# Koellewe/nano-dpow

Hardware: AMD Instinct MI355X
Metric: Gnonce/s blake2b-64 per GPU & 8-GPU node; p50 time-to-work at fffffff8 (higher is better)
Workload: dtype u64

## Files before the change

include/nanopow.h:

```cpp
#ifndef NANOPOW_H
#define NANOPOW_H

#include <stdint.h>

#ifdef __cplusplus
extern "C" {
#endif

#define NPOW_OK 0
#define NPOW_CANCELLED 1
#define NPOW_EXHAUSTED 2
#define NPOW_PENDING 3
#define NPOW_TOO_LATE 4
#define NPOW_ERR_NOT_INITIALISED (-1)
#define NPOW_ERR_NO_DEVICE (-2)
#define NPOW_ERR_BAD_ARGUMENT (-3)
#define NPOW_ERR_HIP (-4)
#define NPOW_ERR_INVALID_WORK (-5)
#define NPOW_ERR_CAPACITY (-6)
#define NPOW_ERR_INTERNAL (-7)

#define NPOW_ABI_VERSION 7

#define NPOW_RESERVE_MIN 0xfffff00000000000ull
// ... 195 lines not shown
  uint64_t launches;
  uint64_t launches_cut;
  uint64_t held_us;
  uint64_t moves;
} npow_range_share_info;

int npow_ticket_share(uint64_t ticket, npow_range_share_info* out);

int npow_values(int device, const uint8_t root[32], uint64_t start, uint64_t count, uint64_t* values_out);

int npow_values_path(int device, const uint8_t root[32], uint64_t start, uint64_t count, int path,
                     uint64_t* values_out);

int npow_values_pairs(int device, const uint8_t* roots, const uint64_t* nonces, uint32_t n,
                      uint64_t* values_out);

int npow_set_tuning(uint32_t iters_per_launch, uint32_t poll_interval, uint32_t blocks_per_cu);

int npow_set_pool_tuning(uint32_t budget_us, uint32_t blocks_per_cu);

int npow_device_stats_get(int device, npow_device_stats* out);
int npow_device_stats_get_sized(int device, npow_device_stats* out, uint64_t size);
int npow_device_stats_reset(int device);

const char* npow_version(void);
int npow_abi_version(void);

#ifdef __cplusplus
}
#endif

#endif
```

nano-dpow_amd/csrc/npow_engine.cpp:

```cpp
#include <hip/hip_runtime.h>

#include <pthread.h>
#include <time.h>

#include <algorithm>
#include <cstddef>
#include <exception>
#include <chrono>
#include <cstdio>
#include <cstdlib>
#include <cstring>
#include <deque>
#include <memory>
#include <mutex>
#include <string>
#include <thread>
#include <vector>

#include "npow_host.h"

namespace npow {

namespace {
thread_local std::string t_err;
// ... 495 lines not shown
  out->stale_missing = d.stale_missing;
  out->stale_gpu_delay_us = d.stale_gpu_delay_us;
  out->linger_ms = d.linger_ms;
  out->promotions = d.promotions;
  return NPOW_OK;
}

int npow_device_stats_get(int device, npow_device_stats* out) try {
  if (!out) return fail(NPOW_ERR_BAD_ARGUMENT, "out is required");
  npow_device_stats full;
  if (int rc = stats_fill(device, &full)) return rc;
  memcpy(out, &full, offsetof(npow_device_stats, kills_relayed));
  return NPOW_OK;
} catch (...) { return guard_exception(); }

int npow_device_stats_get_sized(int device, npow_device_stats* out, uint64_t size) try {
  if (!out || size == 0) return fail(NPOW_ERR_BAD_ARGUMENT, "out and size > 0 are required");
  npow_device_stats full;
  if (int rc = stats_fill(device, &full)) return rc;
  memcpy(out, &full, std::min<uint64_t>(size, sizeof(full)));
  return NPOW_OK;
} catch (...) { return guard_exception(); }

int npow_device_stats_reset(int device) try {
  if (int rc = check_init()) return rc;
  if (device < 0 || device >= (int)g_devs.size()) return fail(NPOW_ERR_BAD_ARGUMENT, "bad device");
  Device& d = *g_devs[device];
  settle_stats(d);
  const double cpu = worker_cpu_ms(d);
  std::lock_guard<std::mutex> g(d.stats_mu);
  d.launches = d.nonces = d.invalid = d.early = d.early_mismatch = d.yields = d.dyn = d.kills_relayed = d.late = 0;
  d.promotions = d.idle_gaps = d.watcher_decisions = d.stale_drains = d.linger_relays = d.stale_late = d.stale_missing = 0;
  d.idle_ms = d.linger_ms = d.stale_gpu_delay_us = 0.0;
  d.kernel_ms = 0.0;
  d.clk_ticks = d.clk_ref_ticks = 0.0;
  d.stats_t0 = std::chrono::steady_clock::now();
  d.worker_cpu0_ms = cpu;
  return NPOW_OK;
} catch (...) { return guard_exception(); }

int npow_search(const uint8_t root[32], uint64_t threshold, uint64_t start, uint64_t device_mask,
                uint64_t max_nonces_per_device, const volatile uint32_t* cancel, uint64_t* nonce_out,
                uint64_t* value_out, uint64_t* nonces_done) try {
  if (int rc = check_init()) return rc;
  if (!root || !nonce_out) return fail(NPOW_ERR_BAD_ARGUMENT, "root and nonce_out are required");
  uint64_t ticket = 0;
  if (int rc = pool_submit(root, threshold, start, device_mask, max_nonces_per_device, cancel, &ticket)) return rc;
  return pool_wait(ticket, -1, nonce_out, value_out, nonces_done);
} catch (...) { return guard_exception(); }

int npow_search_batch(const uint8_t* roots, const uint64_t* thresholds, uint32_t n, uint64_t device_mask,
                      uint64_t max_nonces_per_root, const volatile uint32_t* const* cancel, uint64_t* nonces_out,
                      uint64_t* values_out, int32_t* status_out, uint64_t* nonces_done) try {
  if (int rc = check_init()) return rc;
  if (nonces_done) *nonces_done = 0;
  if (n == 0) return NPOW_OK;
// ... 405 lines not shown
```

nano-dpow_amd/csrc/npow_host.h:

```cpp
#pragma once
#include <hip/hip_runtime.h>
#include <pthread.h>

#include <atomic>
#include <condition_variable>
#include <chrono>
#include <memory>
#include <mutex>
#include <string>
#include <thread>
#include <vector>

#include "../../include/nanopow.h"
#include "npow_blake2b.h"
#include "npow_internal.h"

namespace npow {

int fail(int code, const std::string& msg);
const std::string& last_error();

#define HIPTRY(expr)                                                                        \
  do {                                                                                      \
    hipError_t e_ = (expr);                                                                 \
// ... 17 lines not shown
  HostMailbox* mb_dev = nullptr;
  uint64_t* d_out = nullptr;
  hipEvent_t ev_start[kEventRing] = {};
  hipEvent_t ev_stop[kEventRing] = {};
  std::mutex mu;
  std::atomic<int> tasks_waiting{0};
  PoolDevState* pst = nullptr;
  PoolMailbox* pmb = nullptr;
  PoolMailbox* pmb_dev = nullptr;
  PoolTable* d_tab[kEventRing] = {};
  PoolTable* h_tab[kEventRing] = {};
  unsigned long long* h_done = nullptr;
  hipEvent_t ev_done[kMaxSlots] = {};
  hipStream_t hit_stream = nullptr;
  unsigned long long* h_hit_ring = nullptr;
  unsigned long long* h_hit_n = nullptr;
  uint64_t* h_hits = nullptr;
  std::thread worker;
  std::mutex stats_mu;
  uint64_t launches = 0, nonces = 0, invalid = 0;
  uint64_t early = 0, early_mismatch = 0;
  uint64_t yields = 0, dyn = 0;
  uint64_t linger_ends = 0;
  uint64_t promotions = 0;
  std::atomic<int> counted_inflight{0};
  uint64_t kills_relayed = 0;
  uint64_t late = 0;
  uint64_t watcher_decisions = 0;
  uint64_t stale_drains = 0;
  uint64_t stale_late = 0;
  uint64_t stale_missing = 0;
  double stale_gpu_delay_us = 0.0;
  uint64_t linger_relays = 0;
  double linger_ms = 0.0;
  double idle_ms = 0.0;
  uint64_t idle_gaps = 0;
  std::atomic<bool> worker_busy{false};
  std::atomic<int> active_slots{0};
  std::mutex wake_mu;
  std::condition_variable wake_cv;
  uint64_t wake_seq = 0;
  std::atomic<uint64_t> armed_mask{0};
  std::atomic<uint64_t> armed_gen[kMaxSlots] = {};
  std::atomic<const volatile uint32_t*> armed_cancel[kMaxSlots] = {};
  std::atomic<double> armed_spin_until[kMaxSlots] = {};
  std::mutex armed_mu;
// ... 110 lines not shown
```

nano-dpow_amd/csrc/npow_internal.h:

```cpp
#pragma once
#include <stddef.h>
#include <stdint.h>
#include <hip/hip_runtime.h>

#include "npow_blake2b.h"
#include "npow_weights.h"
#include "npow_claims.h"
#include "npow_dense.h"
#include "npow_hash_asm.inc"
#include "npow_hash_asm_lockstep_ld.inc"

namespace npow {

constexpr int kBlock = 256;
constexpr int kLsWaves = 8;
constexpr int kLsBlock = kLsWaves * 64;
static_assert(kDenseWaves == (uint32_t)kLsWaves, "npow_dense.h: one block per wave of a workgroup");
constexpr int kLsGroups = 4;

enum class Mode : int { kSweep = 1, kValues = 2, kValuesSeq = 3 };

struct LaunchArgs {
  uint64_t u[NPOW_ASM_N_UNIFORMS];
  uint64_t threshold;
// ... 181 lines not shown
  PoolReserve reserve[kMaxSlots];
  alignas(64) uint64_t ctl;
  alignas(64) uint64_t kills;
  alignas(64) PoolClk clk[kPoolRing][kClkWaves];
#ifdef NPOW_DIAG_TIMES
  uint64_t diag_join[1024];
#endif
};

struct PoolShape {
  int grid;
  uint32_t units() const { return (uint32_t)grid; }
  uint64_t own(uint32_t e, uint32_t n, uint32_t iters) const {
    return dense_own(units(), n, e, iters);
  }
  uint64_t full(uint32_t iters) const { return dense_full(units(), iters); }
  uint32_t launch_iters(uint32_t iters) const { return iters > 1 ? iters / 2 : 1u; }
};

hipError_t launch_task(Mode mode, int grid, hipStream_t stream, const LaunchArgs& a, DevState* st,
                       HostMailbox* mb, uint64_t* out);
hipError_t launch_pool(hipStream_t stream, int grid, const PoolTable* tab, bool bounded, PoolDevState* st,
                       PoolMailbox* mb);
hipError_t launch_pool_arg(hipStream_t stream, int grid, const PoolTable& host_tab, bool bounded, PoolDevState* st,
                           PoolMailbox* mb);
inline void fill_uniforms(LaunchArgs& a, const RootPrecomp& pre) { npow_asm_uniforms(pre.m, a.u); }

hipError_t launch_pairs(int grid, hipStream_t stream, const uint64_t* roots_words, const uint64_t* nonces,
                        uint32_t n, uint64_t* out);

}
```

nano-dpow_amd/csrc/npow_kernel.hip:

```cpp
#include <hip/hip_runtime.h>
#include <stdint.h>
#include <string.h>

#include "npow_internal.h"

namespace npow {

__device__ __forceinline__ uint64_t pack(uint32_t lo, uint32_t hi) { return ((uint64_t)hi << 32) | lo; }

__device__ __forceinline__ uint64_t rotr32(uint64_t x) {
  return pack((uint32_t)(x >> 32), (uint32_t)x);
}
template <int N>
__device__ __forceinline__ uint64_t rotr_lt32(uint64_t x) {
  const uint32_t lo = (uint32_t)x, hi = (uint32_t)(x >> 32);
  return pack(__builtin_amdgcn_alignbit(hi, lo, N), __builtin_amdgcn_alignbit(lo, hi, N));
}
__device__ __forceinline__ uint64_t rotr63(uint64_t x) {
  const uint32_t lo = (uint32_t)x, hi = (uint32_t)(x >> 32);
  return pack(__builtin_amdgcn_alignbit(lo, hi, 31), __builtin_amdgcn_alignbit(hi, lo, 31));
}

template <int I>
__device__ __forceinline__ uint64_t add_msg(uint64_t a, uint64_t nonce, const uint64_t (&m)[4]) {
// ... 384 lines not shown
                                             uint64_t wn, uint64_t wv) {
  if (__hip_atomic_fetch_max(&st->slot[slot].dead, (unsigned long long)gen, __ATOMIC_RELAXED,
                             __HIP_MEMORY_SCOPE_AGENT) < gen) {
    PoolWin* pw = &mb->win[slot];
    __hip_atomic_store(&pw->nonce, wn, __ATOMIC_RELAXED, __HIP_MEMORY_SCOPE_SYSTEM);
    __hip_atomic_store(&pw->value, wv, __ATOMIC_RELAXED, __HIP_MEMORY_SCOPE_SYSTEM);
    __hip_atomic_store(&pw->t, __builtin_amdgcn_s_memrealtime(), __ATOMIC_RELAXED, __HIP_MEMORY_SCOPE_SYSTEM);
    __hip_atomic_store(&pw->gen, gen, __ATOMIC_RELEASE, __HIP_MEMORY_SCOPE_SYSTEM);
  }
}

__device__ __forceinline__ void ls2_publish_reserve(PoolDevState* st, PoolMailbox* mb, uint32_t slot, uint64_t gen,
                                                    uint64_t rn, uint64_t rv) {
  const unsigned long long key = pool_reserve_key(gen, rv);
  if (__hip_atomic_fetch_max(&st->reserve_best[slot], key, __ATOMIC_RELAXED, __HIP_MEMORY_SCOPE_AGENT) < key) {
    PoolReserve* pr = &mb->reserve[slot];
    __hip_atomic_store(&pr->nonce, rn, __ATOMIC_RELAXED, __HIP_MEMORY_SCOPE_SYSTEM);
    __hip_atomic_store(&pr->gen, gen, __ATOMIC_RELEASE, __HIP_MEMORY_SCOPE_SYSTEM);
  }
}

constexpr uint32_t kNoEntry = 0xffffffffu;
typedef const __attribute__((address_space(4))) PoolEntry ConstEntry;
__device__ __forceinline__ ConstEntry* ls2_entry(const PoolTable* tab, const PoolMailbox* mb, uint32_t e) {
  const PoolEntry* p = e < tab->n ? &tab->e[e] : &mb->dyn[(tab->dyn_base + (e - tab->n)) % kDynRing].e;
  return (ConstEntry*)(uintptr_t)p;
}
struct EntryHdr {
  uint64_t gen;
  uint32_t slot, bounded, wsh, bg;
};
__device__ __forceinline__ EntryHdr ls2_hdr(const PoolTable* tab, PoolMailbox* mb, uint32_t e) {
  if (e < tab->n) {
    ConstEntry* q = (ConstEntry*)(uintptr_t)&tab->e[e];
    return EntryHdr{q->gen, q->slot, q->bounded, q->wsh, q->bg};
  }
  PoolEntry* q = &mb->dyn[(tab->dyn_base + (e - tab->n)) % kDynRing].e;
  const uint32_t w = __hip_atomic_load(&q->wsh, __ATOMIC_RELAXED, __HIP_MEMORY_SCOPE_SYSTEM);
  return EntryHdr{__hip_atomic_load(&q->gen, __ATOMIC_RELAXED, __HIP_MEMORY_SCOPE_SYSTEM),
                  __hip_atomic_load(&q->slot, __ATOMIC_RELAXED, __HIP_MEMORY_SCOPE_SYSTEM),
                  __hip_atomic_load(&q->bounded, __ATOMIC_RELAXED, __HIP_MEMORY_SCOPE_SYSTEM), w,
                  (w & kWshBg) ? 1u : 0u};
}
__device__ __forceinline__ uint64_t ls2_ctl(PoolMailbox* mb) {
  return __hip_atomic_load(&mb->ctl, __ATOMIC_RELAXED, __HIP_MEMORY_SCOPE_SYSTEM);
}
// ... 354 lines not shown
      if (ok) atomicAdd(&ph->moves[q->slot], 1ull);
    }
    if (__builtin_amdgcn_readfirstlane(ok)) return pick;
  }
  return kNoEntry;
}

__device__ __noinline__ uint32_t ls2_claimed_start(const PoolTable* tab, uint32_t g, uint32_t G, uint32_t csum) {
  const uint32_t lane = __builtin_amdgcn_mbcnt_hi(~0u, __builtin_amdgcn_mbcnt_lo(~0u, 0u));
  const uint32_t n = tab->n < (uint32_t)kMaxSlots ? tab->n : (uint32_t)kMaxSlots;
  const uint32_t r = pool_claimed_pos(g, csum, G, pool_claimed_pad_mult(tab->pad));
  ConstEntry* const le = (ConstEntry*)(uintptr_t)&tab->e[lane < n ? lane : 0u];
  uint32_t acc = lane < n ? 8u >> (le->wsh & 3u) : 0u;
#pragma unroll
  for (int m = 1; m < 64; m <<= 1) {
    const uint32_t o = __shfl_up(acc, m);
    if (lane >= (uint32_t)m) acc += o;
  }
  const uint32_t k = (uint32_t)__builtin_popcountll(__ballot(lane < n && acc <= r));
  return k < n ? k : n - 1u;
}

constexpr uint32_t kPollStride = 0x9E3779B9u;

template <bool BOUNDED>
__device__ __forceinline__ void pool_body_ls2(const PoolTable* __restrict__ tab, PoolDevState* __restrict__ st,
                                              PoolMailbox* __restrict__ mb, const uint64_t t_start) {
  __shared__ uint32_t s_stop[3];
  __shared__ uint32_t s_flag[kLsWaves];
  __shared__ uint32_t s_next;
  __shared__ uint32_t s_done[kLsWaves];
  __shared__ uint32_t s_seen;
  const uint32_t lane = threadIdx.x & 63;
  const uint32_t wv = __builtin_amdgcn_readfirstlane(threadIdx.x >> 6);
  const uint32_t g = blockIdx.x, G = gridDim.x;
  const uint32_t w = g * kLsWaves + wv;
  const uint32_t n = tab->n, iters = tab->iters;
  if (threadIdx.x < 3) s_stop[threadIdx.x] = ~0u;
  const bool counted = tab->counted != 0;
  if (wv == 0) {
    if (lane == 0) {
      s_seen = 0;
      s_over = 0;
    }
    uint32_t first;
    if (n == 0) {
      first = kNoEntry;
    } else if (counted) {
      uint32_t e0 = g % n;
      if constexpr (BOUNDED) {
        const uint32_t cs = pool_claimed_pad_sum(tab->pad);
        if (cs) e0 = ls2_claimed_start(tab, g, G, cs);
      }
      first = ls2_pick(tab, st, mb, e0, true, &s_seen);
    } else {
      ConstEntry* pe = ls2_entry(tab, mb, g % n);
      first = load_dead(st, pe->slot) < pe->gen ? g % n : kNoEntry;
    }
    if (lane == 0) s_next = first;
  }
  __syncthreads();

  uint32_t e = __builtin_amdgcn_readfirstlane(__hip_atomic_load(&s_next, __ATOMIC_RELAXED, __HIP_MEMORY_SCOPE_WORKGROUP));
  uint32_t seg = 0, it = 0;
  uint32_t pc = w;
  bool end = false;
  for (;;) {
  for (;;) {
    if (e == kNoEntry) break;
    const PoolEntry* pe = (const PoolEntry*)ls2_entry(tab, mb, e);
    PoolCursor c;
    pool_load_ls(pe, c, g, wv, G, n, e, iters);
#ifdef NPOW_DIAG_TIMES
    if (wv == 0 && lane == 0) {
      const uint64_t tj = __builtin_amdgcn_s_memrealtime();
      __hip_atomic_store(&mb->fin[c.slot].t_join, tj, __ATOMIC_RELAXED, __HIP_MEMORY_SCOPE_SYSTEM);
      __hip_atomic_store(&mb->diag_join[g & 1023], tj, __ATOMIC_RELAXED, __HIP_MEMORY_SCOPE_SYSTEM);
    }
#endif
    pc = w;
    const uint32_t sw = seg % 3;
    const uint32_t poll_mask = tab->poll_mask, budget = tab->budget;
    unsigned long long* const dead_p = &st->slot[c.slot].dead;
    uint32_t b = it * c.K + c.j;
    uint64_t nonce = c.base + ((uint64_t)b << 6) + lane;
    uint64_t step = (uint64_t)c.K << 6;
    uint32_t done = 0;
    __shared__ uint32_t s_it;
    if constexpr (BOUNDED) {
      if ((c.bounded & kEntryClaim) && wv == 0 && lane == 0) s_it = it;
    }
    for (;;) {
    if constexpr (BOUNDED) {
      if (c.bounded & kEntryClaim) {
        __shared__ uint32_t s_claim;
        if (wv == 0 && lane == 0)
          s_claim = ls2_claim(tab, st, mb, pe,
                              __hip_atomic_load(&s_stop[sw], __ATOMIC_RELAXED, __HIP_MEMORY_SCOPE_WORKGROUP), t_start);
        __syncthreads();
        const uint32_t ci = __builtin_amdgcn_readfirstlane(
            __hip_atomic_load(&s_claim, __ATOMIC_RELAXED, __HIP_MEMORY_SCOPE_WORKGROUP));
        __syncthreads();
        if (ci == kNoEntry) break;
        c.K = kLsWaves;
        c.j = wv;
        step = (uint64_t)kLsWaves << 6;
        it = claim_row_first(ci);
        c.it_end = claim_row_end(c.last_b / kLsWaves + 1u, ci);
        b = it * kLsWaves + wv;
        nonce = c.base + ((uint64_t)b << 6) + lane;
      }
    }
    while (it < c.it_end) {
      const uint32_t verdict = __hip_atomic_load(&s_stop[sw], __ATOMIC_RELAXED, __HIP_MEMORY_SCOPE_WORKGROUP);
      const uint64_t dead = __hip_atomic_load(dead_p, __ATOMIC_RELAXED, __HIP_MEMORY_SCOPE_AGENT);
      const uint32_t v = (uint32_t)__builtin_amdgcn_readfirstlane(verdict);
      if (v != ~0u && (v >> 2) <= it) {
        end = (v & 3u) == 0;
        break;
      }
      const uint32_t it0 = it;
      const uint32_t pc0 = pc;
      const uint64_t thr = c.threshold, gen = c.gen;
      const uint64_t value = npow_asm_work_value_lockstep_ld(nonce, c.up);
      ++it;
      pc += kPollStride;
      bool hit = value >= thr;
      if constexpr (BOUNDED) {
        const uint32_t in_lanes = b < c.last_b ? 64u : (b == c.last_b ? c.tail : 0u);
        hit = hit && lane < in_lanes;
        done += in_lanes;
      } else {
        done += 64;
      }
      uint64_t hits = __ballot(hit);
      if constexpr (BOUNDED) {
        if (__builtin_expect(hits != 0, 0) && (c.bounded & kEntryCollect)) {
          c.threshold = ls2_collect(tab, st, c.up, hits, hit, nonce, value, thr, lane);
          hits = 0;
        }
      }
      uint32_t why = 0u;
      if (__builtin_expect(hits != 0, 0)) {
        ConstEntry* ce = (ConstEntry*)(uintptr_t)c.up;
        asm volatile("" : "+s"(ce));
        const uint32_t wslot = ce->slot;
        const uint64_t wgen = ce->gen;
        PoolFloor* const fl = &mb->floor[wslot];
        const uint64_t fgen = __hip_atomic_load(&fl->gen, __ATOMIC_RELAXED, __HIP_MEMORY_SCOPE_SYSTEM);
        ls2_complete();
        const uint64_t ethr = ce->threshold;
        uint64_t cur = ethr;
        if (uni64(fgen) == wgen) {
          const uint64_t fthr = __hip_atomic_load(&fl->threshold, __ATOMIC_RELAXED, __HIP_MEMORY_SCOPE_SYSTEM);
          ls2_complete();
          cur = uni64(fthr);
        }
        const bool armed = ce->reserve != ethr;
        if (cur > thr) {
          if (!armed) c.threshold = cur;
          const uint64_t keep = hits & __ballot(value >= cur);
          const uint64_t stale = hits & ~keep & __ballot(value >= ethr);
          if (stale != 0 && lane == 0)
            atomicAdd(&st->done[wslot][(blockIdx.x % kPoolDoneShards) * 8 + kStaleWord],
                      (unsigned long long)__builtin_popcountll(stale));
          uint64_t cand = hits & ~keep & ~stale;
          hits = keep;
          if (cand != 0) {
            uint64_t bv = 0, bn = 0;
            do {
              const int cl = __builtin_ctzll(cand);
              cand &= cand - 1;
              const uint64_t cv = readlane64(value, cl);
              if (cv >= bv) {
                bv = cv;
                bn = readlane64(nonce, cl);
              }
            } while (cand != 0);
            if (lane == 0) ls2_publish_reserve(st, mb, wslot, wgen, bn, bv);
          }
        }
        if (hits != 0) {
          why = 2u;
          const int wl = __builtin_ctzll(hits);
          const uint64_t wn = readlane64(nonce, wl), wval = readlane64(value, wl);
          if (lane == 0) ls2_publish_win(st, mb, wslot, wgen, wn, wval);
        }
      }
      if (__builtin_expect((pc0 & poll_mask) == 0, 0)) {
        if (lane == 0) s_flag[wv] = ls2_poll(tab, st, mb, e, &s_seen);
        lds_drain();
        const uint32_t p = __builtin_amdgcn_readfirstlane(
            __hip_atomic_load(&s_flag[wv], __ATOMIC_RELAXED, __HIP_MEMORY_SCOPE_WAVEFRONT));
        why = (p & 2u) ? 2u : (why ? why : (p ? 3u : 0u));
      }
      if (__ballot(dead == gen) != 0) why = 1u;
      const bool late = budget && !c.bounded && (it0 & 3u) == 0 &&
                        (uint32_t)__builtin_amdgcn_s_memrealtime() - (uint32_t)t_start >= budget;
      if (__builtin_expect(why != 0 || late, 0)) {
        if (lane == 0)
          __hip_atomic_fetch_min(&s_stop[sw], (it << 2) | (late ? 0u : why), __ATOMIC_RELAXED,
                                 __HIP_MEMORY_SCOPE_WORKGROUP);
        lds_drain();
      }
      nonce += step;
      b += c.K;
      __builtin_amdgcn_s_barrier();
    }
    if constexpr (BOUNDED) {
      if (c.bounded & kEntryClaim) continue;
    }
    break;
    }
    if (lane == 0) s_done[wv] = done;
    __syncthreads();
    if (wv == 0) {
      uint32_t sum = lane < kLsWaves ? s_done[lane] : 0u;
#pragma unroll
      for (int m = kLsWaves / 2; m >= 1; m >>= 1) sum += __shfl_xor(sum, m);
// ... 12 lines not shown
    if (wv == 0) {
      const uint32_t next = ls2_pick(tab, st, mb, e, false, &s_seen);
      if (lane == 0) {
        s_next = next;
        s_stop[(seg + 1) % 3] = ~0u;
      }
    }
    __syncthreads();
    e = __builtin_amdgcn_readfirstlane(__hip_atomic_load(&s_next, __ATOMIC_RELAXED, __HIP_MEMORY_SCOPE_WORKGROUP));
    ++seg;
  }
  if constexpr (BOUNDED) {
    if (e != kNoEntry || !counted) break;
    __syncthreads();
    if (wv == 0) {
      const uint32_t next = ls2_move_claimed(tab, st, mb, (uint32_t)t_start);
      if (lane == 0) s_next = next;
    }
    __syncthreads();
    e = __builtin_amdgcn_readfirstlane(__hip_atomic_load(&s_next, __ATOMIC_RELAXED, __HIP_MEMORY_SCOPE_WORKGROUP));
    if (e == kNoEntry) break;
    continue;
  }
  if (e != kNoEntry || !tab->linger) break;
  __syncthreads();
  if (wv == 0) {
    const uint32_t next = ls2_linger(tab, st, mb, &s_seen, 0);
    if (lane == 0) s_next = next;
  }
  __syncthreads();
  e = __builtin_amdgcn_readfirstlane(__hip_atomic_load(&s_next, __ATOMIC_RELAXED, __HIP_MEMORY_SCOPE_WORKGROUP));
  if (e == kNoEntry) break;
  }
  if (!counted && wv == 0) ls2_exit(tab, st, mb, G, g);
  clk_end_ls2(tab, mb, t_start, wv);
}

template <bool BOUNDED>
__global__ __launch_bounds__(kLsBlock, 8) void npow_pool_kernel_ls2(const PoolTable* __restrict__ tab,
                                                                   PoolDevState* __restrict__ st,
                                                                   PoolMailbox* __restrict__ mb) {
  uint64_t t_start;
  asm volatile("s_memrealtime %0\n\ts_waitcnt lgkmcnt(0)" : "=s"(t_start) :: "memory");
  clk_begin_lds();
  pool_body_ls2<BOUNDED>(tab, st, mb, t_start);
}

template <bool BOUNDED>
__global__ __launch_bounds__(kLsBlock, 8) void npow_pool_kernel_ls2_arg(const PoolTableArg targ,
                                                                       PoolDevState* __restrict__ st,
                                                                       PoolMailbox* __restrict__ mb) {
  uint64_t t_start;
  asm volatile("s_memrealtime %0\n\ts_waitcnt lgkmcnt(0)" : "=s"(t_start) :: "memory");
  (void)targ;
  const PoolTable* tab = (const PoolTable*)__builtin_amdgcn_kernarg_segment_ptr();
  clk_begin_lds();
  pool_body_ls2<BOUNDED>(tab, st, mb, t_start);
}

hipError_t launch_pool(hipStream_t stream, int grid, const PoolTable* tab, bool bounded, PoolDevState* st,
                       PoolMailbox* mb) {
  if (bounded)
    npow_pool_kernel_ls2<true><<<grid, kLsBlock, 0, stream>>>(tab, st, mb);
  else
    npow_pool_kernel_ls2<false><<<grid, kLsBlock, 0, stream>>>(tab, st, mb);
  return hipGetLastError();
}

hipError_t launch_pool_arg(hipStream_t stream, int grid, const PoolTable& host_tab, bool bounded, PoolDevState* st,
                           PoolMailbox* mb) {
  if (host_tab.n > (uint32_t)kArgEntries) return hipErrorInvalidValue;
  PoolTableArg a;
  memcpy(&a, &host_tab, pool_table_bytes(host_tab.n));
  if (bounded)
    npow_pool_kernel_ls2_arg<true><<<grid, kLsBlock, 0, stream>>>(a, st, mb);
  else
    npow_pool_kernel_ls2_arg<false><<<grid, kLsBlock, 0, stream>>>(a, st, mb);
  return hipGetLastError();
}

__global__ __launch_bounds__(kBlock) void npow_pairs_kernel(const uint64_t* __restrict__ roots_words,
                                                            const uint64_t* __restrict__ nonces, uint32_t n,
                                                            uint64_t* __restrict__ out) {
  const uint32_t i = blockIdx.x * kBlock + threadIdx.x;
  if (i >= n) return;
  uint64_t m[4];
#pragma unroll
  for (int k = 0; k < 4; ++k) m[k] = roots_words[4 * (size_t)i + k];
  out[i] = work_value_full(nonces[i], m);
}

hipError_t launch_task(Mode mode, int grid, hipStream_t stream, const LaunchArgs& a, DevState* st,
                       HostMailbox* mb, uint64_t* out) {
  switch (mode) {
    case Mode::kSweep:
      npow_sweep_kernel_ls2<<<grid, kLsBlock, 0, stream>>>(a, st, mb, out);
      break;
// ... 18 lines not shown
```

nano-dpow_amd/csrc/npow_pool.cpp:

```cpp
#include <hip/hip_runtime.h>
#include <sys/prctl.h>

#include <algorithm>
#include <chrono>
#include <cmath>
#include <condition_variable>
#include <deque>
#include <mutex>
#include <string>
#include <thread>
#include <vector>

#include "npow_pool_impl.h"

namespace npow {
namespace {

constexpr double kYieldMinUs = 1500.0;
constexpr int kYieldMaxLive = 8;
constexpr int kIdleSpinUs = 2000;
constexpr double kPrelaunchUs = 2000.0;
constexpr double kDynMinUs = 3000.0;
constexpr double kFreshSpinUs = 400.0;
constexpr int kInvalidStreakMax = 3;
// ... 274 lines not shown
  uint64_t late_base = 0;
  uint64_t stale_base = 0;
};

struct Counts { uint64_t done, late, stale; };

struct PoolInflight {
  uint64_t seq;
  int ring;
  uint64_t dyn_base;
  uint64_t yield_base;
  bool counted;
  bool linger;
  uint32_t wdown;
  bool bounded;
  struct Collect {
    int slot;
    uint64_t gen;
    uint32_t region, room;
    bool claim;
    uint64_t base, count;
  };
  std::vector<Collect> collect;
  bool claimed() const {
    for (const Collect& c : collect)
      if (c.claim) return true;
    return false;
  }
};

uint64_t collect_span(uint64_t threshold, uint32_t room) {
  const double p = threshold ? (double)(0 - threshold) / 18446744073709551616.0 : 1.0;
  const double fit = (double)room - 8.0 * std::sqrt((double)room) - 64.0;
  const double span = (fit > 64.0 ? fit : 64.0) / p;
  return span >= 9.0e18 ? ~0ull : (uint64_t)span;
}

class Worker {
 public:
  explicit Worker(Device& d) : d_(d) {}
  void run();

 private:
  Device& d_;
  Slot slots_[kMaxSlots];
  std::deque<PoolInflight> q_;
// ... 609 lines not shown

int Worker::launch(bool empty_linger) {
  if (q_.size() >= 2 || d_.dead) return NPOW_OK;
  if (q_.size() == 1 && g_budget_us.load() > 0 && budget_left_us() > kPrelaunchUs && live_slot()) return NPOW_OK;
  uint32_t n = 0;
  int idx[kMaxSlots];
  bool claimed = false;
  for (int s = 0; s < kMaxSlots; ++s)
    if (slots_[s].state == SlotState::kActive && !slots_[s].no_more) {
      idx[n++] = s;
      claimed = claimed || slots_[s].job->held_class();
    }
  if (claimed) n = hold_out(idx, n);
  if (n == 0 && !empty_linger) return NPOW_OK;
  if (!live_slot()) end_linger();
  PoolTable& t = *d_.h_tab[ring_];
  bool bounded = false;
  build_table(t, idx, n, &bounded);
  if (n == 0 && !t.linger) return NPOW_OK;
  const PoolShape sh = pool_shape(d_);
  const int r = ring_;
  ring_ = (ring_ + 1) % kEventRing;
  const size_t bytes = pool_table_bytes(n);
  DEVCHECK(d_, "pool launch");
  if (faults().hip_dev == d_.id && seq_ > faults().hip_after)
    return fail(NPOW_ERR_HIP, "injected launch failure (NANOPOW_FAULT_HIP)");
  if (!collect_.empty())
    HIPTRY(hipMemsetAsync(&d_.pst->hits[r & 1], 0, offsetof(PoolHits, rec), d_.stream));
  if (n <= (uint32_t)kArgEntries) {
    HIPTRY(hipEventRecord(d_.ev_start[r], d_.stream));
    HIPTRY(launch_pool_arg(d_.stream, sh.grid, t, bounded, d_.pst, d_.pmb_dev));
  } else {
    HIPTRY(hipMemcpyAsync(d_.d_tab[r], d_.h_tab[r], bytes, hipMemcpyHostToDevice, d_.stream));
    HIPTRY(hipEventRecord(d_.ev_start[r], d_.stream));
    HIPTRY(launch_pool(d_.stream, sh.grid, d_.d_tab[r], bounded, d_.pst, d_.pmb_dev));
  }
  if (!collect_.empty())
    HIPTRY(hipMemcpyAsync(d_.h_hit_ring + (size_t)r * (offsetof(PoolHits, rec) / sizeof(unsigned long long)),
                          &d_.pst->hits[r & 1], offsetof(PoolHits, rec), hipMemcpyDeviceToHost, d_.stream));
  HIPTRY(hipEventRecord(d_.ev_stop[r], d_.stream));
  if (q_.empty()) front_start_ = std::chrono::steady_clock::now();
  NPOW_DBGT("nanopow[%d]: launch %llu n=%u linger %u wsum %u (weights halved %u times) yield_base %llx slots:", d_.id,
            (unsigned long long)seq_, n, t.linger, t.wsum ? t.wsum : pool_claimed_pad_sum(t.pad), t.wdown, (unsigned long long)t.yield_base);
  for (uint32_t e = 0; e < n; ++e) NPOW_DBG(" %d/g%llu", idx[e], (unsigned long long)t.e[e].gen);
  NPOW_DBG("\n");
  q_.push_back({seq_, r, (uint32_t)ctl_, t.yield_base, t.counted != 0, t.linger != 0, t.wdown, bounded, collect_});
  publish_counted();
  return NPOW_OK;
}

int Worker::queue_readbacks() {
  constexpr size_t row = kPoolDoneShards * 8;
  DEVCHECK(d_, "pool read-back");
  for (int s = 0; s < kMaxSlots; ++s) {
    Slot& sl = slots_[s];
    if (sl.state != SlotState::kDraining || sl.readback || sl.no_readback) continue;
    if (!g_readback_always && !d_.dead) {
      if (sl.early) {
        if (++early_count_ % kVerifyEvery != 0) {
          sl.no_readback = true;
          continue;
        }
      } else if (!sl.fin_seen && sl.stop_us > 0 && !sl.requeue && !sl.inflight.empty() &&
                 now_us() - sl.stop_us < g_linger_us) {
        continue;
      }
    }
    HIPTRY(hipMemcpyAsync(d_.h_done + (size_t)s * row, &d_.pst->done[s][0], row * sizeof(unsigned long long),
                          hipMemcpyDeviceToHost, d_.stream));
// ... 101 lines not shown

void Worker::collect_sweep(Slot& sl, const PoolInflight::Collect& c, const PoolInflight& f, uint64_t n,
                           uint64_t stored) {
  const uint64_t start = sl.job->start;
  std::sort(d_.h_hits, d_.h_hits + stored, [start](uint64_t x, uint64_t y) { return x - start < y - start; });
  std::lock_guard<std::mutex> g(g_pool.mu);
  JobDev& jd = sl.job->dev[sl.k];
  jd.hit_n += n;
  if (n > stored) jd.hits_lost = true;
  const uint64_t take = std::min<uint64_t>(stored, (uint64_t)NPOW_SWEEP_JOB_HITS - jd.hits.size());
  jd.hits.insert(jd.hits.end(), d_.h_hits, d_.h_hits + take);
  jd.launches++;
  if (c.claim) jd.moves += d_.h_hit_n[3 * kMaxSlots + c.slot];
  credit_entry(sl, c, f);
}

int Worker::retire_launches() {
  while (!q_.empty()) {
    const PoolInflight f = q_.front();
    const hipError_t e = hipEventQuery(d_.ev_stop[f.ring]);
    if (e == hipErrorNotReady) break;
    if (e != hipSuccess) return fail(NPOW_ERR_HIP, std::string("pool launch: ") + hipGetErrorString(e));
    account_launch(d_, f.ring);
    if (prev_stop_ring_ >= 0) {
      float gap = 0.f;
      if (hipEventElapsedTime(&gap, d_.ev_stop[prev_stop_ring_], d_.ev_start[f.ring]) == hipSuccess && gap >= 0.f)
        stat([&] { d_.idle_ms += gap; d_.idle_gaps++; });
    }
    prev_stop_ring_ = f.ring;
    uint64_t g0 = 0, g1 = 0;
    account_clock(f.ring, f.seq, &g0, &g1);
    if (g_trace_lat && g0) trace_launch(f, g0, g1);
    if (int rc = collect_hits(f)) return rc;
    for (int s = 0; s < kMaxSlots; ++s) {
      Slot& sl = slots_[s];
      if (sl.state == SlotState::kFree || sl.inflight.empty()) continue;
      if (win_published(s)) handle_win(s);
      size_t m = 0;
      while (m < sl.inflight.size() && sl.inflight[m].seq <= f.seq) ++m;
      if (sl.job && sl.job->max_per_dev && !sl.win_seen && sl.stop_us == 0)
        for (size_t i = 0; i < m; ++i) sl.unread += sl.inflight[i].count;
      sl.inflight.erase(sl.inflight.begin(), sl.inflight.begin() + (ptrdiff_t)m);
      if (sl.inflight.empty()) sl.ending = false;
      if (m > 0 && sl.inflight.empty() && sl.state == SlotState::kDraining && !sl.early && sl.job &&
          sl.job->decided.load()) {
        std::lock_guard<std::mutex> g(g_pool.mu);
// ... 368 lines not shown
```

nano-dpow_amd/csrc/npow_pool_impl.h:

```cpp
#pragma once
#include <cstdio>
#include <cstdlib>
#include <cstring>

#include "npow_pool.h"

namespace npow {

inline const char* env_str(const char* name, const char* dflt) { const char* e = getenv(name); return e ? e : dflt; }
inline double env_num(const char* name, double dflt) { const char* e = getenv(name); return e ? atof(e) : dflt; }
inline const double g_poll_us = env_num("NANOPOW_POLL_US", 50.0);
inline const bool g_debug = getenv("NANOPOW_DEBUG") != nullptr;
inline const int g_linger_env = getenv("NANOPOW_LINGER") ? (getenv("NANOPOW_LINGER")[0] == '0' ? 0 : 1) : -1;
inline const uint32_t g_linger_p = [] {
  uint32_t p = (uint32_t)atoi(env_str("NANOPOW_LINGER_P", "0")), q = 1;
  while (p && q < p) q <<= 1;
  return p ? q : 0u;
}();
inline const double g_linger_us = env_num("NANOPOW_LINGER_US", 1000.0);
inline const bool g_readback_always = strcmp(env_str("NANOPOW_READBACK", ""), "always") == 0;
inline const bool g_watcher_on = strcmp(env_str("NANOPOW_WATCHER", "1"), "0") != 0;
inline const double g_watch_nap_us = env_num("NANOPOW_WATCH_NAP_US", 20.0);
inline const bool g_trace_lat = getenv("NANOPOW_TRACE_LATENCY") != nullptr;
inline const bool g_trace_steps = getenv("NANOPOW_TRACE_STEPS") != nullptr;
inline const bool g_wait_spin = env_str("NANOPOW_WAIT_SPIN", "1")[0] != '0';

struct Faults {
  uint64_t invalid_mask = 0;
  int hip_dev = -1;
  uint64_t hip_after = 0;
  bool retarget_blind = false;
  bool no_moves = false;
};
const Faults& faults();

#define NPOW_DBG(...) \
  do { if (g_debug) fprintf(stderr, __VA_ARGS__); } while (0)
#define NPOW_DBGT(...) \
  do { if (g_debug) fprintf(stderr, "[%.3f] ", now_us() * 1e-3), fprintf(stderr, __VA_ARGS__); } while (0)

void wake_worker(Device& d);

// ... 47 lines not shown
```

nano-dpow_amd/nanopow/_lib.py:

```python
from __future__ import annotations

import ctypes
import os
import threading
import time
from dataclasses import dataclass
from typing import List, Optional, Sequence, Tuple

_HERE = os.path.dirname(os.path.abspath(__file__))
LIB_PATH = os.environ.get("NANOPOW_LIB", os.path.join(_HERE, "libnanopow.so"))

NPOW_OK = 0
NPOW_CANCELLED = 1
NPOW_EXHAUSTED = 2
NPOW_PENDING = 3
NPOW_TOO_LATE = 4
NPOW_ERR_NOT_INITIALISED = -1
NPOW_ERR_NO_DEVICE = -2
NPOW_ERR_BAD_ARGUMENT = -3
NPOW_ERR_HIP = -4
NPOW_ERR_INVALID_WORK = -5
NPOW_ERR_CAPACITY = -6
NPOW_ERR_INTERNAL = -7

NPOW_ABI_VERSION = 7
NPOW_RESERVE_MIN = 0xfffff00000000000
NPOW_PATH_SEARCH = 0
NPOW_PATH_SEQ = 1
NPOW_PATH_GENERIC = 2

NPOW_SWEEP_JOB_HITS = 1 << 20

M64 = (1 << 64) - 1

EXPORTED_SYMBOLS = (
    "npow_init", "npow_shutdown", "npow_last_error", "npow_work_value", "npow_search",
    "npow_search_batch", "npow_sweep", "npow_values", "npow_values_pairs", "npow_set_tuning",
    "npow_device_stats_get", "npow_device_stats_reset", "npow_version",
    "npow_submit", "npow_wait", "npow_cancel", "npow_pool_config", "npow_pool_status",
    "npow_set_pool_tuning", "npow_values_path", "npow_wait_info", "npow_device_stats_get_sized",
    "npow_abi_version", "npow_config_cpu_threads", "npow_wait_result", "npow_submit_weighted",
    "npow_promote", "npow_retarget", "npow_submit_background", "npow_ticket_background",
    "npow_submit_reserve", "npow_ticket_reserve", "npow_relax", "npow_submit_sweep", "npow_wait_sweep",
    "npow_submit_sweep_background", "npow_ticket_sweep", "npow_submit_best", "npow_wait_best", "npow_ticket_best",
    "npow_submit_best_background", "npow_ticket_best_hold",
    "npow_submit_sweep_shared", "npow_submit_best_shared", "npow_ticket_share",
)


class NanoPowError(RuntimeError):
    def __init__(self, code: int, message: str):
        super().__init__(f"nanopow error {code}: {message}")
        self.code = code
        self.message = message


class DeviceStats(ctypes.Structure):
    _fields_ = [
        ("launches", ctypes.c_uint64),
        ("nonces", ctypes.c_uint64),
        ("kernel_ms", ctypes.c_double),
        ("invalid_work", ctypes.c_uint64),
        ("cus", ctypes.c_int32),
        ("grid", ctypes.c_int32),
        ("clock_mhz", ctypes.c_double),
        ("host_cpu_ms", ctypes.c_double),
        ("host_wall_ms", ctypes.c_double),
        ("dead", ctypes.c_int32),
        ("pool_groups", ctypes.c_int32),
# ... 283 lines not shown
        if hasattr(lib, "npow_submit_sweep_background"):
            lib.npow_submit_sweep_background.argtypes = [u8p, u64, u64, u64, u64, p, pu64]
            lib.npow_submit_sweep_background.restype = ctypes.c_int
            lib.npow_ticket_sweep.argtypes = [u64, ctypes.POINTER(_SweepInfoStruct)]
            lib.npow_ticket_sweep.restype = ctypes.c_int
        if hasattr(lib, "npow_submit_best"):
            lib.npow_submit_best.argtypes = [u8p, u64, u64, u64, u64, p, pu64]
            lib.npow_submit_best.restype = ctypes.c_int
            lib.npow_wait_best.argtypes = [u64, ctypes.c_int64, pu64, pu64, pu64]
            lib.npow_wait_best.restype = ctypes.c_int
            lib.npow_ticket_best.argtypes = [u64, ctypes.POINTER(_BestInfoStruct)]
            lib.npow_ticket_best.restype = ctypes.c_int
        if hasattr(lib, "npow_submit_best_background"):
            lib.npow_submit_best_background.argtypes = [u8p, u64, u64, u64, u64, p, pu64]
            lib.npow_submit_best_background.restype = ctypes.c_int
            lib.npow_ticket_best_hold.argtypes = [u64, ctypes.POINTER(_BestHoldStruct)]
            lib.npow_ticket_best_hold.restype = ctypes.c_int
        if hasattr(lib, "npow_submit_sweep_shared"):
            for f in (lib.npow_submit_sweep_shared, lib.npow_submit_best_shared):
                f.argtypes = [u8p, u64, u64, u64, u64, p, pu64]
                f.restype = ctypes.c_int
            lib.npow_ticket_share.argtypes = [u64, ctypes.POINTER(_RangeShareStruct)]
            lib.npow_ticket_share.restype = ctypes.c_int
        _lib = lib
        return lib


def _check(rc: int, lib: ctypes.CDLL, ok=(NPOW_OK,)) -> int:
    if rc in ok:
        return rc
    msg = lib.npow_last_error()
    raise NanoPowError(rc, msg.decode("utf-8", "replace") if msg else "")


def _root(root: bytes) -> bytes:
    if not isinstance(root, (bytes, bytearray)) or len(root) != 32:
        raise ValueError("root must be 32 bytes")
    return bytes(root)


class CancelToken:

    def __init__(self) -> None:
        self._word = ctypes.c_uint32(0)

    def set(self) -> None:
# ... 429 lines not shown
        nn = (ctypes.c_uint64 * max(n, 1))(*[x & M64 for x in nonces])
        out = (ctypes.c_uint64 * max(n, 1))()
        _check(self.lib.npow_values_pairs(device, rb, ctypes.addressof(nn), n, ctypes.addressof(out)), self.lib)
        return list(out[:n])

    def set_tuning(self, iters_per_launch: int = 0, poll_interval: int = 0, blocks_per_cu: int = 0) -> None:
        _check(self.lib.npow_set_tuning(iters_per_launch, poll_interval, blocks_per_cu), self.lib)

    def set_pool_tuning(self, budget_us: Optional[int] = None, blocks_per_cu: int = 0) -> None:
        _check(self.lib.npow_set_pool_tuning(0xffffffff if budget_us is None else budget_us, blocks_per_cu),
               self.lib)

    def set_launch_budget(self, budget_us: int) -> None:
        self.set_pool_tuning(budget_us=budget_us)

    def stats(self, device: int = 0) -> DeviceStats:
        s = DeviceStats()
        if hasattr(self.lib, "npow_device_stats_get_sized"):
            _check(self.lib.npow_device_stats_get_sized(device, ctypes.byref(s), ctypes.sizeof(s)), self.lib)
        else:
            _check(self.lib.npow_device_stats_get(device, ctypes.byref(s)), self.lib)
        return s

    def abi_version(self) -> int:
        return int(self.lib.npow_abi_version())

    def reset_stats(self, device: int = 0) -> None:
        _check(self.lib.npow_device_stats_reset(device), self.lib)

    def version(self) -> str:
        return self.lib.npow_version().decode()


_engine: Optional[Engine] = None
_engine_lock = threading.Lock()


def engine(cpu_threads: int = 0) -> Engine:
    global _engine
    with _engine_lock:
        if _engine is None:
            _engine = Engine(cpu_threads=cpu_threads)
        return _engine
```

Before: 35.03.

## Add specialized one-entry pool kernel with cheaper hit and kill checks

Adds a specialized kernel instantiation for the common case of an unbounded pool launch with a single, uncounted, non-lingering entry. It fixes n=1, drops the counted path and the segment-rotating stop slot, and pre-filters hits with a 32-bit compare on the high word before doing the full 64-bit ballot. It applies the same 32-bit pre-check to the dead-generation test and pads the hot loop to a 128-byte boundary with s_nop. Selection is on by default through NANOPOW_ONE_KERNEL, and a stats counter plus API are added to report how many launches took this path.

```diff
diff --git a/include/nanopow.h b/include/nanopow.h
--- a/include/nanopow.h
+++ b/include/nanopow.h
@@ -241,6 +241,7 @@
 int npow_device_stats_get(int device, npow_device_stats* out);
 int npow_device_stats_get_sized(int device, npow_device_stats* out, uint64_t size);
 int npow_device_stats_reset(int device);
+int npow_device_one_entry_launches(int device, uint64_t* out);
 
 const char* npow_version(void);
 int npow_abi_version(void);
diff --git a/nano-dpow_amd/csrc/npow_engine.cpp b/nano-dpow_amd/csrc/npow_engine.cpp
--- a/nano-dpow_amd/csrc/npow_engine.cpp
+++ b/nano-dpow_amd/csrc/npow_engine.cpp
@@ -541,6 +541,16 @@
   return NPOW_OK;
 } catch (...) { return guard_exception(); }
 
+int npow_device_one_entry_launches(int device, uint64_t* out) try {
+  if (int rc = check_init()) return rc;
+  if (device < 0 || device >= (int)g_devs.size() || !out) return fail(NPOW_ERR_BAD_ARGUMENT, "bad device or out");
+  Device& d = *g_devs[device];
+  settle_stats(d);
+  std::lock_guard<std::mutex> g(d.stats_mu);
+  *out = d.one_launches;
+  return NPOW_OK;
+} catch (...) { return guard_exception(); }
+
 int npow_device_stats_reset(int device) try {
   if (int rc = check_init()) return rc;
   if (device < 0 || device >= (int)g_devs.size()) return fail(NPOW_ERR_BAD_ARGUMENT, "bad device");
@@ -551,6 +561,7 @@
   d.launches = d.nonces = d.invalid = d.early = d.early_mismatch = d.yields = d.dyn = d.kills_relayed = d.late = 0;
   d.promotions = d.idle_gaps = d.watcher_decisions = d.stale_drains = d.linger_relays = d.stale_late = d.stale_missing = 0;
   d.idle_ms = d.linger_ms = d.stale_gpu_delay_us = 0.0;
+  d.one_launches = 0;
   d.kernel_ms = 0.0;
   d.clk_ticks = d.clk_ref_ticks = 0.0;
   d.stats_t0 = std::chrono::steady_clock::now();
diff --git a/nano-dpow_amd/csrc/npow_host.h b/nano-dpow_amd/csrc/npow_host.h
--- a/nano-dpow_amd/csrc/npow_host.h
+++ b/nano-dpow_amd/csrc/npow_host.h
@@ -63,6 +63,7 @@
   uint64_t early = 0, early_mismatch = 0;
   uint64_t yields = 0, dyn = 0;
   uint64_t linger_ends = 0;
+  uint64_t one_launches = 0;
   uint64_t promotions = 0;
   std::atomic<int> counted_inflight{0};
   uint64_t kills_relayed = 0;
diff --git a/nano-dpow_amd/csrc/npow_internal.h b/nano-dpow_amd/csrc/npow_internal.h
--- a/nano-dpow_amd/csrc/npow_internal.h
+++ b/nano-dpow_amd/csrc/npow_internal.h
@@ -227,8 +227,9 @@
                        HostMailbox* mb, uint64_t* out);
 hipError_t launch_pool(hipStream_t stream, int grid, const PoolTable* tab, bool bounded, PoolDevState* st,
                        PoolMailbox* mb);
+bool pool_one_entry(const PoolTable& host_tab, bool bounded);
 hipError_t launch_pool_arg(hipStream_t stream, int grid, const PoolTable& host_tab, bool bounded, PoolDevState* st,
-                           PoolMailbox* mb);
+                           PoolMailbox* mb, bool one = false);
 inline void fill_uniforms(LaunchArgs& a, const RootPrecomp& pre) { npow_asm_uniforms(pre.m, a.u); }
 
 hipError_t launch_pairs(int grid, hipStream_t stream, const uint64_t* roots_words, const uint64_t* nonces,
diff --git a/nano-dpow_amd/csrc/npow_kernel.hip b/nano-dpow_amd/csrc/npow_kernel.hip
--- a/nano-dpow_amd/csrc/npow_kernel.hip
+++ b/nano-dpow_amd/csrc/npow_kernel.hip
@@ -430,6 +430,7 @@
 
 constexpr uint32_t kNoEntry = 0xffffffffu;
 typedef const __attribute__((address_space(4))) PoolEntry ConstEntry;
+typedef __attribute__((address_space(3))) uint32_t lds_u32;
 __device__ __forceinline__ ConstEntry* ls2_entry(const PoolTable* tab, const PoolMailbox* mb, uint32_t e) {
   const PoolEntry* p = e < tab->n ? &tab->e[e] : &mb->dyn[(tab->dyn_base + (e - tab->n)) % kDynRing].e;
   return (ConstEntry*)(uintptr_t)p;
@@ -830,8 +831,9 @@
 }
 
 constexpr uint32_t kPollStride = 0x9E3779B9u;
-
-template <bool BOUNDED>
+constexpr int kOnePad = 6;
+
+template <bool BOUNDED, bool ONE = false>
 __device__ __forceinline__ void pool_body_ls2(const PoolTable* __restrict__ tab, PoolDevState* __restrict__ st,
                                               PoolMailbox* __restrict__ mb, const uint64_t t_start) {
   __shared__ uint32_t s_stop[3];
@@ -843,9 +845,10 @@
   const uint32_t wv = __builtin_amdgcn_readfirstlane(threadIdx.x >> 6);
   const uint32_t g = blockIdx.x, G = gridDim.x;
   const uint32_t w = g * kLsWaves + wv;
-  const uint32_t n = tab->n, iters = tab->iters;
+  static_assert(!(BOUNDED && ONE), "ONE is the unbounded one-entry launch");
+  const uint32_t n = ONE ? 1u : tab->n, iters = tab->iters;
   if (threadIdx.x < 3) s_stop[threadIdx.x] = ~0u;
-  const bool counted = tab->counted != 0;
+  const bool counted = ONE ? false : tab->counted != 0;
   if (wv == 0) {
     if (lane == 0) {
       s_seen = 0;
@@ -887,13 +890,20 @@
     }
 #endif
     pc = w;
-    const uint32_t sw = seg % 3;
+    const uint32_t sw = ONE ? 0u : seg % 3;
     const uint32_t poll_mask = tab->poll_mask, budget = tab->budget;
     unsigned long long* const dead_p = &st->slot[c.slot].dead;
     uint32_t b = it * c.K + c.j;
     uint64_t nonce = c.base + ((uint64_t)b << 6) + lane;
     uint64_t step = (uint64_t)c.K << 6;
     uint32_t done = 0;
+    lds_u32* stop_p = (lds_u32*)&s_stop[sw];
+    uint32_t thr_hi = 0, gen_lo = 0;
+    if constexpr (ONE) {
+      asm volatile("" : "+v"(stop_p));
+      thr_hi = __builtin_amdgcn_readfirstlane((uint32_t)(c.threshold >> 32));
+      gen_lo = __builtin_amdgcn_readfirstlane((uint32_t)c.gen);
+    }
     __shared__ uint32_t s_it;
     if constexpr (BOUNDED) {
       if ((c.bounded & kEntryClaim) && wv == 0 && lane == 0) s_it = it;
@@ -919,8 +929,15 @@
         nonce = c.base + ((uint64_t)b << 6) + lane;
       }
     }
+    if constexpr (ONE) {
+      asm volatile(".p2align 7\n\t.rept %0\n\ts_nop 0\n\t.endr" ::"n"(kOnePad));
+    }
     while (it < c.it_end) {
-      const uint32_t verdict = __hip_atomic_load(&s_stop[sw], __ATOMIC_RELAXED, __HIP_MEMORY_SCOPE_WORKGROUP);
+      uint32_t verdict;
+      if constexpr (ONE)
+        verdict = __hip_atomic_load(stop_p, __ATOMIC_RELAXED, __HIP_MEMORY_SCOPE_WORKGROUP);
+      else
+        verdict = __hip_atomic_load(&s_stop[sw], __ATOMIC_RELAXED, __HIP_MEMORY_SCOPE_WORKGROUP);
       const uint64_t dead = __hip_atomic_load(dead_p, __ATOMIC_RELAXED, __HIP_MEMORY_SCOPE_AGENT);
       const uint32_t v = (uint32_t)__builtin_amdgcn_readfirstlane(verdict);
       if (v != ~0u && (v >> 2) <= it) {
@@ -941,7 +958,13 @@
       } else {
         done += 64;
       }
-      uint64_t hits = __ballot(hit);
+      uint64_t hits;
+      if constexpr (ONE) {
+        hits = __ballot((uint32_t)(value >> 32) >= thr_hi);
+        if (__builtin_expect(hits != 0, 0)) hits = __ballot(hit);
+      } else {
+        hits = __ballot(hit);
+      }
       if constexpr (BOUNDED) {
         if (__builtin_expect(hits != 0, 0) && (c.bounded & kEntryCollect)) {
           c.threshold = ls2_collect(tab, st, c.up, hits, hit, nonce, value, thr, lane);
@@ -966,7 +989,10 @@
         }
         const bool armed = ce->reserve != ethr;
         if (cur > thr) {
-          if (!armed) c.threshold = cur;
+          if (!armed) {
+            c.threshold = cur;
+            if constexpr (ONE) thr_hi = __builtin_amdgcn_readfirstlane((uint32_t)(cur >> 32));
+          }
           const uint64_t keep = hits & __ballot(value >= cur);
           const uint64_t stale = hits & ~keep & __ballot(value >= ethr);
           if (stale != 0 && lane == 0)
@@ -1002,7 +1028,11 @@
             __hip_atomic_load(&s_flag[wv], __ATOMIC_RELAXED, __HIP_MEMORY_SCOPE_WAVEFRONT));
         why = (p & 2u) ? 2u : (why ? why : (p ? 3u : 0u));
       }
-      if (__ballot(dead == gen) != 0) why = 1u;
+      if constexpr (ONE) {
+        if (__builtin_expect(__ballot((uint32_t)dead == gen_lo) != 0, 0) && __ballot(dead == gen) != 0) why = 1u;
+      } else {
+        if (__ballot(dead == gen) != 0) why = 1u;
+      }
       const bool late = budget && !c.bounded && (it0 & 3u) == 0 &&
                         (uint32_t)__builtin_amdgcn_s_memrealtime() - (uint32_t)t_start >= budget;
       if (__builtin_expect(why != 0 || late, 0)) {
@@ -1061,7 +1091,7 @@
     if (e == kNoEntry) break;
     continue;
   }
-  if (e != kNoEntry || !tab->linger) break;
+  if (ONE || e != kNoEntry || !tab->linger) break;
   __syncthreads();
   if (wv == 0) {
     const uint32_t next = ls2_linger(tab, st, mb, &s_seen, 0);
@@ -1097,6 +1127,17 @@
   pool_body_ls2<BOUNDED>(tab, st, mb, t_start);
 }
 
+__global__ __launch_bounds__(kLsBlock, 8) void npow_search1_kernel_arg(const PoolTableArg targ,
+                                                                      PoolDevState* __restrict__ st,
+                                                                      PoolMailbox* __restrict__ mb) {
+  uint64_t t_start;
+  asm volatile("s_memrealtime %0\n\ts_waitcnt lgkmcnt(0)" : "=s"(t_start) :: "memory");
+  (void)targ;
+  const PoolTable* tab = (const PoolTable*)__builtin_amdgcn_kernarg_segment_ptr();
+  clk_begin_lds();
+  pool_body_ls2<false, true>(tab, st, mb, t_start);
+}
+
 hipError_t launch_pool(hipStream_t stream, int grid, const PoolTable* tab, bool bounded, PoolDevState* st,
                        PoolMailbox* mb) {
   if (bounded)
@@ -1106,12 +1147,19 @@
   return hipGetLastError();
 }
 
+bool pool_one_entry(const PoolTable& host_tab, bool bounded) {
+  return !bounded && host_tab.n == 1 && !host_tab.counted && !host_tab.linger;
+}
+
 hipError_t launch_pool_arg(hipStream_t stream, int grid, const PoolTable& host_tab, bool bounded, PoolDevState* st,
-                           PoolMailbox* mb) {
+                           PoolMailbox* mb, bool one) {
   if (host_tab.n > (uint32_t)kArgEntries) return hipErrorInvalidValue;
+  if (one && !pool_one_entry(host_tab, bounded)) return hipErrorInvalidValue;
   PoolTableArg a;
   memcpy(&a, &host_tab, pool_table_bytes(host_tab.n));
-  if (bounded)
+  if (one)
+    npow_search1_kernel_arg<<<grid, kLsBlock, 0, stream>>>(a, st, mb);
+  else if (bounded)
     npow_pool_kernel_ls2_arg<true><<<grid, kLsBlock, 0, stream>>>(a, st, mb);
   else
     npow_pool_kernel_ls2_arg<false><<<grid, kLsBlock, 0, stream>>>(a, st, mb);
diff --git a/nano-dpow_amd/csrc/npow_pool.cpp b/nano-dpow_amd/csrc/npow_pool.cpp
--- a/nano-dpow_amd/csrc/npow_pool.cpp
+++ b/nano-dpow_amd/csrc/npow_pool.cpp
@@ -320,6 +320,7 @@
     uint64_t base, count;
   };
   std::vector<Collect> collect;
+  bool one = false;
   bool claimed() const {
     for (const Collect& c : collect)
       if (c.claim) return true;
@@ -975,6 +976,7 @@
   const int r = ring_;
   ring_ = (ring_ + 1) % kEventRing;
   const size_t bytes = pool_table_bytes(n);
+  bool one = false;
   DEVCHECK(d_, "pool launch");
   if (faults().hip_dev == d_.id && seq_ > faults().hip_after)
     return fail(NPOW_ERR_HIP, "injected launch failure (NANOPOW_FAULT_HIP)");
@@ -982,7 +984,8 @@
     HIPTRY(hipMemsetAsync(&d_.pst->hits[r & 1], 0, offsetof(PoolHits, rec), d_.stream));
   if (n <= (uint32_t)kArgEntries) {
     HIPTRY(hipEventRecord(d_.ev_start[r], d_.stream));
-    HIPTRY(launch_pool_arg(d_.stream, sh.grid, t, bounded, d_.pst, d_.pmb_dev));
+    one = g_one_kernel && pool_one_entry(t, bounded);
+    HIPTRY(launch_pool_arg(d_.stream, sh.grid, t, bounded, d_.pst, d_.pmb_dev, one));
   } else {
     HIPTRY(hipMemcpyAsync(d_.d_tab[r], d_.h_tab[r], bytes, hipMemcpyHostToDevice, d_.stream));
     HIPTRY(hipEventRecord(d_.ev_start[r], d_.stream));
@@ -997,7 +1000,7 @@
             (unsigned long long)seq_, n, t.linger, t.wsum ? t.wsum : pool_claimed_pad_sum(t.pad), t.wdown, (unsigned long long)t.yield_base);
   for (uint32_t e = 0; e < n; ++e) NPOW_DBG(" %d/g%llu", idx[e], (unsigned long long)t.e[e].gen);
   NPOW_DBG("\n");
-  q_.push_back({seq_, r, (uint32_t)ctl_, t.yield_base, t.counted != 0, t.linger != 0, t.wdown, bounded, collect_});
+  q_.push_back({seq_, r, (uint32_t)ctl_, t.yield_base, t.counted != 0, t.linger != 0, t.wdown, bounded, collect_, one});
   publish_counted();
   return NPOW_OK;
 }
@@ -1145,6 +1148,10 @@
     if (e == hipErrorNotReady) break;
     if (e != hipSuccess) return fail(NPOW_ERR_HIP, std::string("pool launch: ") + hipGetErrorString(e));
     account_launch(d_, f.ring);
+    if (f.one) {
+      std::lock_guard<std::mutex> g(d_.stats_mu);
+      d_.one_launches++;
+    }
     if (prev_stop_ring_ >= 0) {
       float gap = 0.f;
       if (hipEventElapsedTime(&gap, d_.ev_stop[prev_stop_ring_], d_.ev_start[f.ring]) == hipSuccess && gap >= 0.f)
diff --git a/nano-dpow_amd/csrc/npow_pool_impl.h b/nano-dpow_amd/csrc/npow_pool_impl.h
--- a/nano-dpow_amd/csrc/npow_pool_impl.h
+++ b/nano-dpow_amd/csrc/npow_pool_impl.h
@@ -18,6 +18,7 @@
   return p ? q : 0u;
 }();
 inline const double g_linger_us = env_num("NANOPOW_LINGER_US", 1000.0);
+inline const bool g_one_kernel = env_str("NANOPOW_ONE_KERNEL", "1")[0] != '0';
 inline const bool g_readback_always = strcmp(env_str("NANOPOW_READBACK", ""), "always") == 0;
 inline const bool g_watcher_on = strcmp(env_str("NANOPOW_WATCHER", "1"), "0") != 0;
 inline const double g_watch_nap_us = env_num("NANOPOW_WATCH_NAP_US", 20.0);
diff --git a/nano-dpow_amd/nanopow/_lib.py b/nano-dpow_amd/nanopow/_lib.py
--- a/nano-dpow_amd/nanopow/_lib.py
+++ b/nano-dpow_amd/nanopow/_lib.py
@@ -45,6 +45,7 @@
     "npow_submit_sweep_background", "npow_ticket_sweep", "npow_submit_best", "npow_wait_best", "npow_ticket_best",
     "npow_submit_best_background", "npow_ticket_best_hold",
     "npow_submit_sweep_shared", "npow_submit_best_shared", "npow_ticket_share",
+    "npow_device_one_entry_launches",
 )
 
 
@@ -374,6 +375,9 @@
                 f.restype = ctypes.c_int
             lib.npow_ticket_share.argtypes = [u64, ctypes.POINTER(_RangeShareStruct)]
             lib.npow_ticket_share.restype = ctypes.c_int
+        if hasattr(lib, "npow_device_one_entry_launches"):
+            lib.npow_device_one_entry_launches.argtypes = [ctypes.c_int, pu64]
+            lib.npow_device_one_entry_launches.restype = ctypes.c_int
         _lib = lib
         return lib
 
@@ -849,6 +853,12 @@
             _check(self.lib.npow_device_stats_get(device, ctypes.byref(s)), self.lib)
         return s
 
+    def one_entry_launches(self, device: int = 0) -> int:
+        _JobTicket._need(self.lib, "npow_device_one_entry_launches")
+        n = ctypes.c_uint64(0)
+        _check(self.lib.npow_device_one_entry_launches(device, ctypes.byref(n)), self.lib)
+        return n.value
+
     def abi_version(self) -> int:
         return int(self.lib.npow_abi_version())
 
```

New measurement: 35.02. Within noise of the previous version (-0.0%).
